# OpenDriveLab/ViDAR

Measured on AMD Instinct MI355X. Metric: train samples/sec (6-cam->BEV step), higher is better.
Workload: dtype f32

## Files before the change

### vidar_amd/csrc/gemm_mfma.hip

```cpp
#include <hip/hip_runtime.h>

#include <stdint.h>

#include "vidar_hip.h"
#include "vidar_common.h"

namespace {

typedef __bf16 bf16x8 __attribute__((ext_vector_type(8)));
typedef __bf16 bf16x2 __attribute__((ext_vector_type(2)));
typedef float f32x16 __attribute__((ext_vector_type(16)));
typedef float f32x2 __attribute__((ext_vector_type(2)));
typedef float f32x4 __attribute__((ext_vector_type(4)));
typedef float f32x4u __attribute__((ext_vector_type(4), aligned(4)));
typedef uint32_t u32x4 __attribute__((ext_vector_type(4)));
typedef uint32_t u32x2 __attribute__((ext_vector_type(2)));

constexpr int BM = 128, BN = 128, THREADS = 256;
constexpr int BK = 32;
constexpr int MN_STRIDE = 128 + 8;
template <int PREC>
struct Geo {
  static constexpr int UNITS = (PREC == 1) ? 16 : 32;
  static constexpr int KM_STRIDE = (PREC == 1) ? UNITS : UNITS + 4;
  static constexpr int IMG_DWORDS = (128 * KM_STRIDE > UNITS * MN_STRIDE) ? 128 * KM_STRIDE : UNITS * MN_STRIDE;
  static constexpr int NS = UNITS / 8;
};
constexpr int PREC_F32 = 0, PREC_BF16X3 = 1;
constexpr int LAY_K = 0, LAY_MN = 1;

struct GemmArgs {
  const float* A; const float* B; float* C;
  int64_t lda, ldb, ldc, sA, sB, sC;
  int M, N, K;
  int splits, k_chunk;
  int slabs;
  const float* scale; const float* shift; int vec_axis;
  const float* residual; int64_t ldr, sR;
  int relu;
  int tiles_m, tiles_n, m_fastest;
  int total;
  float* a_rowsum;
  float* rowsum_ws;
};

template <int PREC>
struct Staged {
  static constexpr int CH = 2;
  f32x4 v[CH][2];
};

template <int PREC>
struct KMap {
  static constexpr int LPR = 8;
  static constexpr int RPI = 64 / LPR;
  static constexpr int NI = 32 / RPI;
};

typedef uint32_t raw4 __attribute__((__vector_size__(4 * sizeof(uint32_t))));

__device__ __forceinline__ __amdgpu_buffer_rsrc_t make_rsrc(const float* p, int64_t bytes = 0x7fffffff) {
  const uint64_t a = (uint64_t)p;
  const uint32_t lo = __builtin_amdgcn_readfirstlane((uint32_t)a), hi = __builtin_amdgcn_readfirstlane((uint32_t)(a >> 32));
  const int32_t n = __builtin_amdgcn_readfirstlane((int32_t)(bytes > 0x7fffffff ? 0x7fffffff : bytes));
  return __builtin_amdgcn_make_buffer_rsrc((void*)(((uint64_t)hi << 32) | lo), 0, n, 0x00020000);
}
__device__ __forceinline__ f32x4 ld16(__amdgpu_buffer_rsrc_t r, uint32_t voff, uint32_t soff) {
  return __builtin_bit_cast(f32x4, __builtin_amdgcn_raw_buffer_load_b128(r, voff, soff, 0));
}
__device__ __forceinline__ float ld4(__amdgpu_buffer_rsrc_t r, uint32_t voff, uint32_t soff) {
  return __builtin_bit_cast(float, __builtin_amdgcn_raw_buffer_load_b32(r, voff, soff, 0));
}

template <int PREC>
__device__ __forceinline__ uint32_t voff_kmajor(int64_t ld, int tid) {
  using M = KMap<PREC>;
  const int lane = tid & 63, wave = tid >> 6;
  return (uint32_t)(((32 * wave + lane / M::LPR) * (uint32_t)ld + (lane % M::LPR) * 4) * 4);
}

template <int PREC>
__device__ __forceinline__ void load_kmajor(Staged<PREC>& s, __amdgpu_buffer_rsrc_t rs, int64_t ld, int krel, int k0, int kend,
                                            bool tail, int tid, uint32_t voff) {
  using M = KMap<PREC>;
#pragma unroll
  for (int i = 0; i < M::NI; ++i)
    s.v[i >> 1][i & 1] = ld16(rs, voff, (uint32_t)((i * M::RPI * (uint32_t)ld + krel) * 4));
  if (tail) {
    const int k = k0 + ((tid & 63) % M::LPR) * 4;
#pragma unroll
    for (int i = 0; i < M::NI; ++i)
#pragma unroll
      for (int j = 0; j < 4; ++j) s.v[i >> 1][i & 1][j] = (k + j < kend) ? s.v[i >> 1][i & 1][j] : 0.0f;
  }
}

template <int PREC>
__device__ __forceinline__ uint32_t voff_mnmajor(int64_t ld, int tid) {
  const int kr = (PREC == PREC_BF16X3) ? (tid >> 5) * 2 : (tid >> 5);
  return (uint32_t)((kr * (uint32_t)ld + (tid & 31) * 4) * 4);
}

template <int PREC>
__device__ __forceinline__ void load_mnmajor(Staged<PREC>& s, __amdgpu_buffer_rsrc_t rs, int64_t ld, int krel, uint32_t voff) {
#pragma unroll
  for (int i = 0; i < Staged<PREC>::CH * 2; ++i) {
    const int ku = (PREC == PREC_BF16X3) ? 16 * (i >> 1) + (i & 1) : 8 * i;
    s.v[i >> 1][i & 1] = ld16(rs, voff, (uint32_t)(krel + ku) * (uint32_t)ld * 4u);
  }
}

__device__ __forceinline__ void split2(float a, float b, uint32_t& hi, uint32_t& lo) {
  f32x2 x = {a, b};
  bf16x2 h = __builtin_convertvector(x, bf16x2);
  f32x2 r = x - __builtin_convertvector(h, f32x2);
  bf16x2 l = __builtin_convertvector(r, bf16x2);
  hi = __builtin_bit_cast(uint32_t, h);
  lo = __builtin_bit_cast(uint32_t, l);
}

template <int PREC>
__device__ __forceinline__ void store_kmajor(const Staged<PREC>& s, uint32_t* img, int tid) {
  using M = KMap<PREC>;
  const int lane = tid & 63, wave = tid >> 6;
  const int r0 = 32 * wave + lane / M::LPR, kq = lane % M::LPR;
#pragma unroll
  for (int i = 0; i < M::NI; ++i) {
    const int r = r0 + i * M::RPI;
    const f32x4 v = s.v[i >> 1][i & 1];
    if (PREC == PREC_BF16X3) {
      uint32_t h0, l0, h1, l1;
      split2(v[0], v[1], h0, l0);
      split2(v[2], v[3], h1, l1);
      const int pos = r * Geo<PREC>::KM_STRIDE + ((((kq >> 1) ^ ((r >> 2) & 3)) << 2) | ((kq & 1) << 1));
      *(u32x2*)(img + pos) = u32x2{h0, h1};
      *(u32x2*)(img + Geo<PREC>::IMG_DWORDS + pos) = u32x2{l0, l1};
    } else {
      *(u32x4*)(img + r * Geo<PREC>::KM_STRIDE + 4 * kq) = __builtin_bit_cast(u32x4, v);
    }
  }
}

template <int PREC>
__device__ __forceinline__ void store_mnmajor(const Staged<PREC>& s, uint32_t* img, int tid) {
  if (PREC == PREC_BF16X3) {
#pragma unroll
    for (int c = 0; c < 2; ++c) {
      const int item = tid + 256 * c;
      const int cq = (item & 31) * 4, u = item >> 5;
      u32x4 hi, lo;
#pragma unroll
      for (int j = 0; j < 4; ++j) {
        uint32_t h, l;
        split2(s.v[c][0][j], s.v[c][1][j], h, l);
        hi[j] = h; lo[j] = l;
      }
      *(u32x4*)(img + u * MN_STRIDE + cq) = hi;
      *(u32x4*)(img + Geo<PREC>::IMG_DWORDS + u * MN_STRIDE + cq) = lo;
    }
  } else {
#pragma unroll
    for (int i = 0; i < 4; ++i) {
      const int item = tid + 256 * i;
      *(u32x4*)(img + (item >> 5) * MN_STRIDE + (item & 31) * 4) = __builtin_bit_cast(u32x4, s.v[i >> 1][i & 1]);
    }
  }
}

template <int PREC, int LAY>
__device__ __forceinline__ u32x4 frag(const uint32_t* img, int row, int s, int h) {
  if (LAY == LAY_K) {
    if (PREC == PREC_BF16X3)
      return *(const u32x4*)(img + row * Geo<PREC>::KM_STRIDE + (((2 * s + h) ^ ((row >> 2) & 3)) << 2));
    return *(const u32x4*)(img + row * Geo<PREC>::KM_STRIDE + 8 * s + 4 * h);
  }
  u32x4 f;
  const uint32_t* p = img + (8 * s + 4 * h) * MN_STRIDE + row;
#pragma unroll
  for (int j = 0; j < 4; ++j) f[j] = p[j * MN_STRIDE];
  return f;
}

struct Tile {
  int z, batch, m0, n0, kbeg, kend;
  __amdgpu_buffer_rsrc_t rsA, rsB;
};

template <int PREC, int ALAY, int BLAY>
__device__ __forceinline__ Tile decode_tile(const GemmArgs& g, int t) {
  const int per_z = g.tiles_m * g.tiles_n;
  int id;
  {
    const int q = g.total >> 3, r = g.total & 7, x = t & 7;
    id = (x < r ? x * (q + 1) : r * (q + 1) + (x - r) * q) + (t >> 3);
  }
  Tile T;
  T.z = __builtin_amdgcn_readfirstlane(id / per_z);
  const int tt = id - T.z * per_z;
  const int tm = __builtin_amdgcn_readfirstlane(g.m_fastest ? tt % g.tiles_m : tt / g.tiles_n);
  const int tn = __builtin_amdgcn_readfirstlane(g.m_fastest ? tt / g.tiles_m : tt % g.tiles_n);
  T.batch = __builtin_amdgcn_readfirstlane(T.z / g.splits);
  const int split = T.z - T.batch * g.splits;
  T.m0 = tm * BM; T.n0 = tn * BN;
  T.kbeg = split * g.k_chunk;
  T.kend = min(g.K, T.kbeg + g.k_chunk);
  const float* A = g.A + (int64_t)T.batch * g.sA;
  const float* B = g.B + (int64_t)T.batch * g.sB;
  const int64_t kleft = g.K - T.kbeg;
  T.rsA = ALAY == LAY_K ? make_rsrc(A + (int64_t)T.m0 * g.lda + T.kbeg, ((int64_t)(g.M - 1 - T.m0) * g.lda + kleft) * 4)
                        : make_rsrc(A + (int64_t)T.kbeg * g.lda + T.m0, ((kleft - 1) * g.lda + (g.M - T.m0)) * 4);
  T.rsB = BLAY == LAY_K ? make_rsrc(B + (int64_t)T.n0 * g.ldb + T.kbeg, ((int64_t)(g.N - 1 - T.n0) * g.ldb + kleft) * 4)
                        : make_rsrc(B + (int64_t)T.kbeg * g.ldb + T.n0, ((kleft - 1) * g.ldb + (g.N - T.n0)) * 4);
  return T;
}

template <int PREC, int ALAY, int BLAY>
__device__ __forceinline__ void fetch(Staged<PREC>& sa, Staged<PREC>& sb, const GemmArgs& g, const Tile& T, int k0, int tid,
                                      uint32_t voa, uint32_t vob) {
  const int krel = k0 - T.kbeg;
  const bool tail = k0 + BK > T.kend;
  if (ALAY == LAY_K) load_kmajor<PREC>(sa, T.rsA, g.lda, krel, k0, T.kend, tail, tid, voa);
  else load_mnmajor<PREC>(sa, T.rsA, g.lda, krel, voa);
  if (BLAY == LAY_K) load_kmajor<PREC>(sb, T.rsB, g.ldb, krel, k0, T.kend, tail, tid, vob);
  else load_mnmajor<PREC>(sb, T.rsB, g.ldb, krel, vob);
}

template <int PREC>
__device__ __forceinline__ void add_rowsum(f32x4& rs, const Staged<PREC>& sa) {
#pragma unroll
  for (int i = 0; i < Staged<PREC>::CH * 2; ++i) rs += sa.v[i >> 1][i & 1];
}

template <int PREC, int ALAY, int BLAY>
__device__ __forceinline__ void mainloop(f32x16 (&acc)[2][2], Staged<PREC>& sa, Staged<PREC>& sb, const GemmArgs& g,
                                         const Tile& T, uint32_t* imgA, uint32_t* imgB, int tid, uint32_t voa, uint32_t vob,
                                         f32x4& rowsum, bool want_rowsum) {
  constexpr int IMGS = (PREC == PREC_BF16X3) ? 2 : 1;
  constexpr int IMG_DWORDS = Geo<PREC>::IMG_DWORDS;
  const int lane = tid & 63, wave = tid >> 6;
  const int wm = (wave >> 1) * 64, wn = (wave & 1) * 64;
  const int l31 = lane & 31, h = lane >> 5;
  for (int k0 = T.kbeg; k0 < T.kend; k0 += BK) {
    if (ALAY == LAY_MN && want_rowsum) add_rowsum<PREC>(rowsum, sa);
    if (ALAY == LAY_K) store_kmajor<PREC>(sa, imgA, tid); else store_mnmajor<PREC>(sa, imgA, tid);
    if (BLAY == LAY_K) store_kmajor<PREC>(sb, imgB, tid); else store_mnmajor<PREC>(sb, imgB, tid);
    __syncthreads();
    if (k0 + BK < T.kend) fetch<PREC, ALAY, BLAY>(sa, sb, g, T, k0 + BK, tid, voa, vob);
#pragma unroll
    for (int s = 0; s < Geo<PREC>::NS; ++s) {
      u32x4 fa[2][IMGS], fb[2][IMGS];
#pragma unroll
      for (int i = 0; i < 2; ++i)
#pragma unroll
        for (int p = 0; p < IMGS; ++p) {
          fa[i][p] = frag<PREC, ALAY>(imgA + p * IMG_DWORDS, wm + 32 * i + l31, s, h);
          fb[i][p] = frag<PREC, BLAY>(imgB + p * IMG_DWORDS, wn + 32 * i + l31, s, h);
        }
      if (PREC == PREC_BF16X3) {
#pragma unroll
        for (int term = 0; term < 3; ++term)
#pragma unroll
          for (int i = 0; i < 2; ++i)
#pragma unroll
            for (int j = 0; j < 2; ++j) {
              const bf16x8 a = __builtin_bit_cast(bf16x8, fa[i][term == 0 ? IMGS - 1 : 0]);
              const bf16x8 b = __builtin_bit_cast(bf16x8, fb[j][term == 1 ? IMGS - 1 : 0]);
              acc[i][j] = __builtin_amdgcn_mfma_f32_32x32x16_bf16(a, b, acc[i][j], 0, 0, 0);
            }
      } else {
#pragma unroll
        for (int u = 0; u < 4; ++u)
#pragma unroll
          for (int i = 0; i < 2; ++i)
#pragma unroll
            for (int j = 0; j < 2; ++j) {
              const f32x4 bf = __builtin_bit_cast(f32x4, fb[j][0]), af = __builtin_bit_cast(f32x4, fa[i][0]);
              acc[i][j] = __builtin_amdgcn_mfma_f32_32x32x2f32(af[u], bf[u], acc[i][j], 0, 0, 0);
            }
      }
    }
    __syncthreads();
  }
}

template <bool RAGGED_M>
__device__ __forceinline__ void epilogue_impl(const f32x16 (&acc)[2][2], const GemmArgs& g, const Tile& T, int tid) {
  const int lane = tid & 63, wave = tid >> 6;
  const int wm = (wave >> 1) * 64, wn = (wave & 1) * 64;
  const int l31 = lane & 31, h = lane >> 5;
  const int m0 = T.m0, n0 = T.n0;
  float* C; int64_t ldc;
  if (g.slabs) { C = g.C + (int64_t)T.z * g.M * g.N; ldc = g.N; }
  else { C = g.C + (int64_t)T.batch * g.sC; ldc = g.ldc; }
  const bool epi = !g.slabs;
  const bool by_n = epi && g.vec_axis == 0, by_m = epi && g.vec_axis == 1;
  const int rows_left = g.M - m0, cols_left = g.N - n0;
  const int mleft = rows_left - wm - 4 * h;
  const __amdgpu_buffer_rsrc_t rsC = make_rsrc(C + (int64_t)m0 * ldc + n0, ((int64_t)(rows_left - 1) * ldc + cols_left) * 4);
  const uint32_t voC = (uint32_t)(((wm + 4 * h) * (uint32_t)ldc + wn + l31) * 4);
  const bool has_res = epi && g.residual != nullptr;
  const float* Rp = has_res ? g.residual + (int64_t)T.batch * g.sR + (int64_t)m0 * g.ldr + n0 : C;
  const __amdgpu_buffer_rsrc_t rsR = make_rsrc(Rp, has_res ? ((int64_t)(rows_left - 1) * g.ldr + cols_left) * 4 : 0);
  const uint32_t voR = (uint32_t)(((wm + 4 * h) * (uint32_t)g.ldr + wn + l31) * 4);
  const bool m_scale = by_m && g.scale != nullptr, m_shift = by_m && g.shift != nullptr;
  const __amdgpu_buffer_rsrc_t rsS = make_rsrc(m_scale ? g.scale + m0 : C, m_scale ? (int64_t)rows_left * 4 : 0);
  const __amdgpu_buffer_rsrc_t rsH = make_rsrc(m_shift ? g.shift + m0 : C, m_shift ? (int64_t)rows_left * 4 : 0);
  const uint32_t voM = (uint32_t)((wm + 4 * h) * 4);
#pragma unroll
  for (int j = 0; j < 2; ++j) {
    const int n = n0 + wn + 32 * j + l31;
    if (n >= g.N) continue;
    float sn = 1.0f, bn = 0.0f;
    if (by_n && g.scale) sn = g.scale[n];
    if (by_n && g.shift) bn = g.shift[n];
#pragma unroll
    for (int i = 0; i < 2; ++i) {
#pragma unroll
      for (int r0 = 0; r0 < 16; r0 += 8) {
        float sc[8], sh[8], rs[8];
#pragma unroll
        for (int r = 0; r < 8; ++r) {
          const int row = 32 * i + (r & 3) + 8 * ((r0 + r) >> 2);
          sc[r] = m_scale ? ld4(rsS, voM, (uint32_t)(row * 4)) : sn;
          sh[r] = m_shift ? ld4(rsH, voM, (uint32_t)(row * 4)) : bn;
          rs[r] = has_res ? ld4(rsR, voR, (uint32_t)((row * (uint32_t)g.ldr + 32 * j) * 4)) : 0.0f;
        }
#pragma unroll
        for (int r = 0; r < 8; ++r) {
          const int row = 32 * i + (r & 3) + 8 * ((r0 + r) >> 2);
          float y = acc[i][j][r0 + r];
          if (epi) {
            y = y * sc[r] + sh[r] + rs[r];
            if (g.relu && !(y > 0.0f)) y = 0.0f;
          }
          if (!RAGGED_M || row < mleft)
            __builtin_amdgcn_raw_buffer_store_b32(__builtin_bit_cast(uint32_t, y), rsC, voC,
                                                    (uint32_t)((row * (uint32_t)ldc + 32 * j) * 4), 0);
        }
      }
    }
  }
}

__device__ __forceinline__ void epilogue(const f32x16 (&acc)[2][2], const GemmArgs& g, const Tile& T, int tid) {
  if (g.M - T.m0 >= BM) epilogue_impl<false>(acc, g, T, tid);
  else epilogue_impl<true>(acc, g, T, tid);
}

template <int PREC, int ALAY, int BLAY>
__global__ __launch_bounds__(THREADS, 3) void gemm_mfma_kernel(GemmArgs g) {
  constexpr int IMGS = (PREC == PREC_BF16X3) ? 2 : 1;
  __shared__ __attribute__((aligned(16))) uint32_t lds[2 * IMGS * Geo<PREC>::IMG_DWORDS];
  uint32_t* imgA = lds;
  uint32_t* imgB = lds + IMGS * Geo<PREC>::IMG_DWORDS;
  const int tid = threadIdx.x;
  const uint32_t voa = ALAY == LAY_K ? voff_kmajor<PREC>(g.lda, tid) : voff_mnmajor<PREC>(g.lda, tid);
  const uint32_t vob = BLAY == LAY_K ? voff_kmajor<PREC>(g.ldb, tid) : voff_mnmajor<PREC>(g.ldb, tid);
  Staged<PREC> sa, sb;
  int t = blockIdx.x;
  if (t >= g.total) return;
  Tile cur = decode_tile<PREC, ALAY, BLAY>(g, t);
  if (cur.kbeg < cur.kend) fetch<PREC, ALAY, BLAY>(sa, sb, g, cur, cur.kbeg, tid, voa, vob);
  for (;;) {
    f32x16 acc[2][2];
#pragma unroll
    for (int i = 0; i < 2; ++i)
#pragma unroll
      for (int j = 0; j < 2; ++j)
#pragma unroll
        for (int r = 0; r < 16; ++r) acc[i][j][r] = 0.0f;
    f32x4 rowsum = {0.f, 0.f, 0.f, 0.f};
    const bool want_rowsum = ALAY == LAY_MN && g.a_rowsum != nullptr && cur.n0 == 0;
    mainloop<PREC, ALAY, BLAY>(acc, sa, sb, g, cur, imgA, imgB, tid, voa, vob, rowsum, want_rowsum);
    if (want_rowsum) {
      float* red = reinterpret_cast<float*>(lds);
      const int quad = tid & 31, part = tid >> 5;
      *(f32x4*)(red + (part * 32 + quad) * 4) = rowsum;
      __syncthreads();
      if (tid < BM) {
        float sum = 0.f;
#pragma unroll
        for (int p8 = 0; p8 < 8; ++p8) sum += red[(p8 * 32 + (tid >> 2)) * 4 + (tid & 3)];
        if (cur.m0 + tid < g.M) g.rowsum_ws[(int64_t)cur.z * g.M + cur.m0 + tid] = sum;
      }
      __syncthreads();
    }
    const int tn = t + (int)gridDim.x;
    const bool more = tn < g.total;
    if (more) {
      const Tile nxt = decode_tile<PREC, ALAY, BLAY>(g, tn);
      if (nxt.kbeg < nxt.kend) fetch<PREC, ALAY, BLAY>(sa, sb, g, nxt, nxt.kbeg, tid, voa, vob);
    }
    epilogue(acc, g, cur, tid);
    if (!more) break;
    cur = decode_tile<PREC, ALAY, BLAY>(g, tn);
    t = tn;
  }
}

constexpr int WS_THREADS = 512;

__device__ __forceinline__ void lds_barrier() { asm volatile("s_waitcnt lgkmcnt(0)\n\ts_barrier" ::: "memory"); }

template <int PREC, int ALAY, int BLAY>
struct Cursor {
  int t;
  int k0;
  Tile T;
  __device__ __forceinline__ void start(const GemmArgs& g, int t0) {
    t = t0;
    while (t < g.total) {
      T = decode_tile<PREC, ALAY, BLAY>(g, t);
      if (T.kbeg < T.kend) break;
      t += (int)gridDim.x;
    }
    k0 = (t < g.total) ? T.kbeg : 0;
  }
  __device__ __forceinline__ bool valid(const GemmArgs& g) const { return t < g.total; }
  __device__ __forceinline__ void advance(const GemmArgs& g) {
    k0 += BK;
    if (k0 >= T.kend) start(g, t + (int)gridDim.x);
  }
};

template <int PREC, int ALAY, int BLAY>
__global__ __launch_bounds__(WS_THREADS, 2) void gemm_mfma_ws_kernel(GemmArgs g) {
  constexpr int IMGS = (PREC == PREC_BF16X3) ? 2 : 1;
  constexpr int IMG_DWORDS = Geo<PREC>::IMG_DWORDS;
  constexpr int STAGE_DWORDS = 2 * IMGS * IMG_DWORDS;
  __shared__ __attribute__((aligned(16))) uint32_t lds[2 * STAGE_DWORDS];
  const int tid = threadIdx.x;
  const int wave = __builtin_amdgcn_readfirstlane(tid >> 6);
  if ((int)blockIdx.x >= g.total) return;

  if (wave >= 4) {
    const int ptid = tid - 256;
    const uint32_t voa = ALAY == LAY_K ? voff_kmajor<PREC>(g.lda, ptid) : voff_mnmajor<PREC>(g.lda, ptid);
    const uint32_t vob = BLAY == LAY_K ? voff_kmajor<PREC>(g.ldb, ptid) : voff_mnmajor<PREC>(g.ldb, ptid);
    Staged<PREC> sa0, sb0, sa1, sb1;
    Cursor<PREC, ALAY, BLAY> rd;
    rd.start(g, (int)blockIdx.x);
    int steps = 0;
    for (int t = (int)blockIdx.x; t < g.total; t += (int)gridDim.x) {
      const Tile T = decode_tile<PREC, ALAY, BLAY>(g, t);
      steps += (T.kend > T.kbeg) ? (T.kend - T.kbeg + BK - 1) / BK : 0;
    }
    if (rd.valid(g)) { fetch<PREC, ALAY, BLAY>(sa0, sb0, g, rd.T, rd.k0, ptid, voa, vob); rd.advance(g); }
    if (rd.valid(g)) { fetch<PREC, ALAY, BLAY>(sa1, sb1, g, rd.T, rd.k0, ptid, voa, vob); rd.advance(g); }
    for (int gs = 0; gs < steps; gs += 2) {
      {
        uint32_t* imgA = lds;
        uint32_t* imgB = lds + IMGS * IMG_DWORDS;
        if (ALAY == LAY_K) store_kmajor<PREC>(sa0, imgA, ptid); else store_mnmajor<PREC>(sa0, imgA, ptid);
        if (BLAY == LAY_K) store_kmajor<PREC>(sb0, imgB, ptid); else store_mnmajor<PREC>(sb0, imgB, ptid);
        if (rd.valid(g)) { fetch<PREC, ALAY, BLAY>(sa0, sb0, g, rd.T, rd.k0, ptid, voa, vob); rd.advance(g); }
        lds_barrier();
      }
      if (gs + 1 < steps) {
        uint32_t* imgA = lds + STAGE_DWORDS;
        uint32_t* imgB = lds + STAGE_DWORDS + IMGS * IMG_DWORDS;
        if (ALAY == LAY_K) store_kmajor<PREC>(sa1, imgA, ptid); else store_mnmajor<PREC>(sa1, imgA, ptid);
        if (BLAY == LAY_K) store_kmajor<PREC>(sb1, imgB, ptid); else store_mnmajor<PREC>(sb1, imgB, ptid);
        if (rd.valid(g)) { fetch<PREC, ALAY, BLAY>(sa1, sb1, g, rd.T, rd.k0, ptid, voa, vob); rd.advance(g); }
        lds_barrier();
      }
    }
    return;
  }

  const int lane = tid & 63;
  const int wm = (wave >> 1) * 64, wn = (wave & 1) * 64;
  const int l31 = lane & 31, h = lane >> 5;
  int gs = 0;
  for (int t = (int)blockIdx.x; t < g.total; t += (int)gridDim.x) {
    const Tile T = decode_tile<PREC, ALAY, BLAY>(g, t);
    f32x16 acc[2][2];
#pragma unroll
    for (int i = 0; i < 2; ++i)
#pragma unroll
      for (int j = 0; j < 2; ++j)
#pragma unroll
        for (int r = 0; r < 16; ++r) acc[i][j][r] = 0.0f;
    for (int k0 = T.kbeg; k0 < T.kend; k0 += BK, ++gs) {
      lds_barrier();
      const uint32_t* imgA = lds + (gs & 1) * STAGE_DWORDS;
      const uint32_t* imgB = imgA + IMGS * IMG_DWORDS;
#pragma unroll
      for (int s = 0; s < Geo<PREC>::NS; ++s) {
        u32x4 fa[2][IMGS], fb[2][IMGS];
#pragma unroll
        for (int i = 0; i < 2; ++i)
#pragma unroll
          for (int p = 0; p < IMGS; ++p) {
            fa[i][p] = frag<PREC, ALAY>(imgA + p * IMG_DWORDS, wm + 32 * i + l31, s, h);
            fb[i][p] = frag<PREC, BLAY>(imgB + p * IMG_DWORDS, wn + 32 * i + l31, s, h);
          }
        if (PREC == PREC_BF16X3) {
#pragma unroll
          for (int term = 0; term < 3; ++term)
#pragma unroll
            for (int i = 0; i < 2; ++i)
#pragma unroll
              for (int j = 0; j < 2; ++j) {
                const bf16x8 a = __builtin_bit_cast(bf16x8, fa[i][term == 0 ? IMGS - 1 : 0]);
                const bf16x8 b = __builtin_bit_cast(bf16x8, fb[j][term == 1 ? IMGS - 1 : 0]);
                acc[i][j] = __builtin_amdgcn_mfma_f32_32x32x16_bf16(a, b, acc[i][j], 0, 0, 0);
              }
        } else {
#pragma unroll
          for (int u = 0; u < 4; ++u)
#pragma unroll
            for (int i = 0; i < 2; ++i)
#pragma unroll
              for (int j = 0; j < 2; ++j) {
                const f32x4 bf = __builtin_bit_cast(f32x4, fb[j][0]), af = __builtin_bit_cast(f32x4, fa[i][0]);
                acc[i][j] = __builtin_amdgcn_mfma_f32_32x32x2f32(af[u], bf[u], acc[i][j], 0, 0, 0);
              }
        }
      }
    }
    epilogue(acc, g, T, tid);
  }
}

__global__ __launch_bounds__(256) void gemm_slab_reduce_kernel(const float* __restrict__ ws, int Z, GemmArgs g) {
  __shared__ f32x4 part[4][64];
  if (g.a_rowsum != nullptr) {
    const int lane = threadIdx.x & 63;
    for (int m = (int)blockIdx.x * 4 + (threadIdx.x >> 6); m < g.M; m += (int)gridDim.x * 4) {
      float a = 0.f;
      for (int z = lane; z < Z; z += 64) a += g.rowsum_ws[(int64_t)z * g.M + m];
#pragma unroll
      for (int off = 32; off > 0; off >>= 1) a += __shfl_xor(a, off, 64);
      if (lane == 0) g.a_rowsum[m] = a;
    }
  }
  const int64_t total = (int64_t)g.M * g.N;
  const int64_t quads = total >> 2;
  const int col = threadIdx.x & 63, zg = threadIdx.x >> 6;
  for (int64_t q0 = (int64_t)blockIdx.x * 64; q0 < quads + 1; q0 += (int64_t)gridDim.x * 64) {
    const int64_t q = q0 + col;
    f32x4 a = {0.f, 0.f, 0.f, 0.f};
    if (q < quads) {
      for (int z = zg; z < Z; z += 4) a += *(const f32x4u*)(ws + (int64_t)z * total + 4 * q);
    } else if (q == quads) {
      for (int z = zg; z < Z; z += 4)
        for (int e = 0; e < (int)(total & 3); ++e) a[e] += ws[(int64_t)z * total + 4 * q + e];
    }
    part[zg][col] = a;
    __syncthreads();
    if (zg == 0 && q <= quads) {
      const f32x4 sum = ((part[0][col] + part[1][col]) + part[2][col]) + part[3][col];
      const int n_el = q < quads ? 4 : (int)(total & 3);
      for (int e = 0; e < n_el; ++e) {
        const int64_t idx = 4 * q + e;
        const int m = (int)(idx / g.N), n = (int)(idx - (int64_t)m * g.N);
        const int vi = g.vec_axis == 1 ? m : n;
        float y = sum[e] * (g.scale ? g.scale[vi] : 1.0f) + (g.shift ? g.shift[vi] : 0.0f);
        if (g.residual) y += g.residual[(int64_t)m * g.ldr + n];
        g.C[(int64_t)m * g.ldc + n] = (g.relu && !(y > 0.0f)) ? 0.0f : y;
      }
    }
    __syncthreads();
  }
}

template <int PREC>
void launch_ws(const GemmArgs& g, int a_layout, int b_layout, dim3 grid, hipStream_t st) {
  if (a_layout == LAY_K && b_layout == LAY_K) hipLaunchKernelGGL((gemm_mfma_ws_kernel<PREC, LAY_K, LAY_K>), grid, dim3(WS_THREADS), 0, st, g);
  else if (a_layout == LAY_K) hipLaunchKernelGGL((gemm_mfma_ws_kernel<PREC, LAY_K, LAY_MN>), grid, dim3(WS_THREADS), 0, st, g);
  else if (b_layout == LAY_K) hipLaunchKernelGGL((gemm_mfma_ws_kernel<PREC, LAY_MN, LAY_K>), grid, dim3(WS_THREADS), 0, st, g);
  else hipLaunchKernelGGL((gemm_mfma_ws_kernel<PREC, LAY_MN, LAY_MN>), grid, dim3(WS_THREADS), 0, st, g);
}

int g_gemm_variant = 0;

template <int PREC>
void launch(const GemmArgs& g, int a_layout, int b_layout, dim3 grid, hipStream_t st) {
  if (a_layout == LAY_K && b_layout == LAY_K) hipLaunchKernelGGL((gemm_mfma_kernel<PREC, LAY_K, LAY_K>), grid, dim3(THREADS), 0, st, g);
  else if (a_layout == LAY_K) hipLaunchKernelGGL((gemm_mfma_kernel<PREC, LAY_K, LAY_MN>), grid, dim3(THREADS), 0, st, g);
  else if (b_layout == LAY_K) hipLaunchKernelGGL((gemm_mfma_kernel<PREC, LAY_MN, LAY_K>), grid, dim3(THREADS), 0, st, g);
  else hipLaunchKernelGGL((gemm_mfma_kernel<PREC, LAY_MN, LAY_MN>), grid, dim3(THREADS), 0, st, g);
}

int num_cus() {
  static int cached[64] = {0};
  int dev = 0;
  if (hipGetDevice(&dev) != hipSuccess || dev < 0 || dev >= 64) return 256;
  if (cached[dev] == 0) {
    hipDeviceProp_t prop;
    cached[dev] = (hipGetDeviceProperties(&prop, dev) == hipSuccess && prop.multiProcessorCount > 0)
                      ? prop.multiProcessorCount : 256;
  }
  return cached[dev];
}

int pick_splits(int M, int N, int K, int batch, int bk) {
  const int tiles = ((M + BM - 1) / BM) * ((N + BN - 1) / BN) * batch;
  int s = (512 + tiles - 1) / tiles;
  const int max_s = (K + 4 * bk - 1) / (4 * bk);
  if (s > max_s) s = max_s;
  if (s < 1) s = 1;
  if (s > 256) s = 256;
  return s;
}

}

extern "C" {

int vidar_gemm_set_variant(int variant) {
  const int prev = g_gemm_variant;
  g_gemm_variant = (variant < 0 || variant > 2) ? 0 : variant;
  return prev;
}

int vidar_gemm_splits(int M, int N, int K, int batch, int precision, int reduce) {
  if (!reduce) return 1;
  return pick_splits(M, N, K, batch, BK);
}

size_t vidar_gemm_workspace_bytes(int M, int N, int K, int batch, int precision, int reduce) {
  if (!reduce) return 0;
  const int s = vidar_gemm_splits(M, N, K, batch, precision, reduce);
  const size_t Z = (size_t)batch * s;
  if (reduce == 1) return Z > 1 ? Z * (size_t)M * N * sizeof(float) : 0;
  return Z * ((size_t)M * N + M) * sizeof(float);
}

int vidar_gemm_f32(const float* A, int64_t lda, int a_layout, const float* B, int64_t ldb, int b_layout, float* C,
                   int64_t ldc, int M, int N, int K, int batch, int64_t strideA, int64_t strideB, int64_t strideC,
                   const float* scale, const float* shift, int vec_axis, const float* residual, int64_t ldr,
                   int64_t strideR, int relu, int precision, int reduce, float* a_rowsum, void* workspace,
                   size_t workspace_bytes, void* stream) {
  VIDAR_ENTER();
  if (a_rowsum != nullptr && !(reduce && a_layout == LAY_MN)) return VIDAR_ERR_BAD_ARG;
  if (A == nullptr || B == nullptr || C == nullptr || M <= 0 || N <= 0 || K <= 0 || batch <= 0) return VIDAR_ERR_BAD_ARG;
  if ((a_layout != LAY_K && a_layout != LAY_MN) || (b_layout != LAY_K && b_layout != LAY_MN)) return VIDAR_ERR_BAD_ARG;
  if (precision != PREC_F32 && precision != PREC_BF16X3) return VIDAR_ERR_BAD_ARG;
  if (vec_axis != 0 && vec_axis != 1) return VIDAR_ERR_BAD_ARG;
  if (lda < (a_layout == LAY_K ? K : M) || ldb < (b_layout == LAY_K ? K : N) || ldc < N) return VIDAR_ERR_BAD_ARG;
  if (residual != nullptr && (ldr < N || ldr >= (1 << 22))) return VIDAR_ERR_BAD_ARG;
  if (ldc >= (1 << 22)) return VIDAR_ERR_BAD_ARG;
  if (lda >= (1 << 22) || ldb >= (1 << 22)) return VIDAR_ERR_BAD_ARG;
  if ((a_layout == LAY_MN && (int64_t)K * lda >= (1LL << 29)) || (b_layout == LAY_MN && (int64_t)K * ldb >= (1LL << 29)))
    return VIDAR_ERR_BAD_ARG;
  hipStream_t st = (hipStream_t)stream;
  const int bk = BK;
  GemmArgs g;
  g.A = A; g.B = B; g.C = C;
  g.lda = lda; g.ldb = ldb; g.ldc = ldc; g.sA = strideA; g.sB = strideB; g.sC = strideC;
  g.M = M; g.N = N; g.K = K;
  g.scale = scale; g.shift = shift; g.vec_axis = vec_axis; g.residual = residual; g.ldr = ldr; g.sR = strideR;
  g.relu = relu;
  g.tiles_m = (M + BM - 1) / BM; g.tiles_n = (N + BN - 1) / BN;
  g.m_fastest = M < N;
  g.splits = reduce ? pick_splits(M, N, K, batch, bk) : 1;
  g.k_chunk = ((K + g.splits - 1) / g.splits + bk - 1) / bk * bk;
  const int Z = batch * g.splits;
  g.slabs = (reduce && (Z > 1 || a_rowsum != nullptr)) ? 1 : 0;
  g.a_rowsum = a_rowsum;
  g.rowsum_ws = nullptr;
  if ((int64_t)g.tiles_m * g.tiles_n * Z > 0x3fffffff) return VIDAR_ERR_BAD_ARG;
  g.total = g.tiles_m * g.tiles_n * Z;
  if (reduce && (strideC != 0 || strideR != 0) && batch > 1) return VIDAR_ERR_BAD_ARG;
  GemmArgs k = g;
  if (g.slabs) {
    const size_t need = (size_t)Z * ((size_t)M * N + (a_rowsum ? M : 0)) * sizeof(float);
    if (workspace == nullptr || workspace_bytes < need) return VIDAR_ERR_BAD_ARG;
    k.C = (float*)workspace;
    g.rowsum_ws = a_rowsum ? (float*)workspace + (size_t)Z * M * N : nullptr;
    k.rowsum_ws = g.rowsum_ws;
  }
  k.total = g.tiles_m * g.tiles_n * Z;
  if (g_gemm_variant >= 1 && a_rowsum == nullptr) {
    const int resident = num_cus() * g_gemm_variant / 8 * 8;
    dim3 grid(k.total > resident ? resident : k.total);
    if (precision == PREC_BF16X3) launch_ws<PREC_BF16X3>(k, a_layout, b_layout, grid, st);
    else launch_ws<PREC_F32>(k, a_layout, b_layout, grid, st);
  } else {
    const int resident = num_cus() * 3 / 8 * 8;
    dim3 grid(k.total > resident ? resident : k.total);
    if (precision == PREC_BF16X3) launch<PREC_BF16X3>(k, a_layout, b_layout, grid, st);
    else launch<PREC_F32>(k, a_layout, b_layout, grid, st);
  }
  if (g.slabs) {
    const int64_t total = (int64_t)M * N;
    int blocks = (int)((total / 4 + 1 + 63) / 64);
    if (blocks > 4096) blocks = 4096;
    hipLaunchKernelGGL(gemm_slab_reduce_kernel, dim3(blocks), dim3(256), 0, st, (const float*)workspace, Z, g);
  }
  return vidar_last_error();
}

}
```

Before: 2.925.

## Overlap last K-step MFMAs with epilogue stores in persistent f32 GEMM

```diff
diff --git a/vidar_amd/csrc/gemm_mfma.hip b/vidar_amd/csrc/gemm_mfma.hip
--- a/vidar_amd/csrc/gemm_mfma.hip
+++ b/vidar_amd/csrc/gemm_mfma.hip
@@ -233,14 +233,14 @@
 
 template <int PREC, int ALAY, int BLAY>
 __device__ __forceinline__ void mainloop(f32x16 (&acc)[2][2], Staged<PREC>& sa, Staged<PREC>& sb, const GemmArgs& g,
-                                         const Tile& T, uint32_t* imgA, uint32_t* imgB, int tid, uint32_t voa, uint32_t vob,
-                                         f32x4& rowsum, bool want_rowsum) {
+                                         const Tile& T, int kstop, uint32_t* imgA, uint32_t* imgB, int tid, uint32_t voa,
+                                         uint32_t vob, f32x4& rowsum, bool want_rowsum) {
   constexpr int IMGS = (PREC == PREC_BF16X3) ? 2 : 1;
   constexpr int IMG_DWORDS = Geo<PREC>::IMG_DWORDS;
   const int lane = tid & 63, wave = tid >> 6;
   const int wm = (wave >> 1) * 64, wn = (wave & 1) * 64;
   const int l31 = lane & 31, h = lane >> 5;
-  for (int k0 = T.kbeg; k0 < T.kend; k0 += BK) {
+  for (int k0 = T.kbeg; k0 < kstop; k0 += BK) {
     if (ALAY == LAY_MN && want_rowsum) add_rowsum<PREC>(rowsum, sa);
     if (ALAY == LAY_K) store_kmajor<PREC>(sa, imgA, tid); else store_mnmajor<PREC>(sa, imgA, tid);
     if (BLAY == LAY_K) store_kmajor<PREC>(sb, imgB, tid); else store_mnmajor<PREC>(sb, imgB, tid);
@@ -347,10 +347,92 @@
   else epilogue_impl<true>(acc, g, T, tid);
 }
 
+constexpr int TAB_DWORDS = 2 * (BM + BM);
+
+__device__ __forceinline__ void lds_barrier() { asm volatile("s_waitcnt lgkmcnt(0)\n\ts_barrier" ::: "memory"); }
+
+__device__ __forceinline__ bool piped_tile(const GemmArgs& g, const Tile& T) {
+  return !g.slabs && (g.vec_axis == 1 || (g.scale == nullptr && g.shift == nullptr)) && g.M - T.m0 >= BM &&
+         g.N - T.n0 >= BN && T.kbeg < T.kend;
+}
+
+__device__ __forceinline__ float table_value(const GemmArgs& g, const Tile& T, int tid) {
+  const float* v = tid < BM ? g.scale : g.shift;
+  float x = tid < BM ? 1.0f : 0.0f;
+  if (v != nullptr) x = v[T.m0 + (tid & (BM - 1))];
+  return x;
+}
+
+template <int ALAY, int BLAY>
+__device__ __forceinline__ void last_step_stage(const Staged<PREC_F32>& sa, const Staged<PREC_F32>& sb, uint32_t* imgA,
+                                                uint32_t* imgB, float* tab, float tabv, int tid) {
+  if (ALAY == LAY_K) store_kmajor<PREC_F32>(sa, imgA, tid); else store_mnmajor<PREC_F32>(sa, imgA, tid);
+  if (BLAY == LAY_K) store_kmajor<PREC_F32>(sb, imgB, tid); else store_mnmajor<PREC_F32>(sb, imgB, tid);
+  tab[tid] = tabv;
+  __syncthreads();
+}
+
+template <int ALAY, int BLAY>
+__device__ __forceinline__ void last_step_piped(f32x16 (&acc)[2][2], const GemmArgs& g, const Tile& T, const uint32_t* imgA,
+                                                const uint32_t* imgB, const float* tab, int tid0) {
+  constexpr int PREC = PREC_F32;
+  int tid = tid0;
+  asm volatile("" : "+v"(tid));
+  const int lane = tid & 63, wave = tid >> 6;
+  const int wm = (wave >> 1) * 64, wn = (wave & 1) * 64;
+  const int l31 = lane & 31, h = lane >> 5;
+  const __amdgpu_buffer_rsrc_t rsC = make_rsrc(g.C + (int64_t)T.batch * g.sC + (int64_t)T.m0 * g.ldc + T.n0,
+                                               ((int64_t)(BM - 1) * g.ldc + BN) * 4);
+  const uint32_t ldc = (uint32_t)g.ldc, ldr = (uint32_t)g.ldr;
+  const uint32_t voC = (uint32_t)(((wm + 4 * h) * ldc + wn + l31) * 4);
+  const bool has_res = g.residual != nullptr;
+  const __amdgpu_buffer_rsrc_t rsR =
+      make_rsrc(has_res ? g.residual + (int64_t)T.batch * g.sR + (int64_t)T.m0 * g.ldr + T.n0 : g.C,
+                has_res ? ((int64_t)(BM - 1) * g.ldr + BN) * 4 : 0);
+  const uint32_t voR = (uint32_t)(((wm + 4 * h) * ldr + wn + l31) * 4), voRz = has_res ? voR : 0u;
+  const uint32_t rb = has_res ? 4u : 0u;
+  const float* tsc = tab + wm + 4 * h;
+  const float* tsh = tsc + BM;
+  const bool relu = g.relu != 0;
+  float rs[16];
+#pragma unroll
+  for (int r = 0; r < 16; ++r) rs[r] = ld4(rsR, voRz, (uint32_t)((((r & 3) + 8 * (r >> 2)) * ldr) * rb));
+  __builtin_amdgcn_sched_barrier(0);
+#pragma unroll
+  for (int sub = 0; sub <= 4; ++sub) {
+    const int i = (sub >> 1) & 1, j = sub & 1;
+    const int pi = ((sub - 1) >> 1) & 1, pj = (sub - 1) & 1;
+    asm volatile("" ::: "memory");
+#pragma unroll
+    for (int s = 0; s < 4; ++s) {
+      f32x4 af = {0.f, 0.f, 0.f, 0.f}, bf = af;
+      if (sub < 4) {
+        af = __builtin_bit_cast(f32x4, frag<PREC, ALAY>(imgA, wm + 32 * i + l31, s, h));
+        bf = __builtin_bit_cast(f32x4, frag<PREC, BLAY>(imgB, wn + 32 * j + l31, s, h));
+      }
+#pragma unroll
+      for (int u = 0; u < 4; ++u) {
+        if (sub < 4) acc[i][j] = __builtin_amdgcn_mfma_f32_32x32x2f32(af[u], bf[u], acc[i][j], 0, 0, 0);
+        if (sub > 0) {
+          const int r = 4 * s + u;
+          const int prow = 32 * pi + 8 * s + u;
+          float y = acc[pi][pj][r] * tsc[prow] + tsh[prow] + rs[r];
+          if (relu && !(y > 0.0f)) y = 0.0f;
+          __builtin_amdgcn_raw_buffer_store_b32(__builtin_bit_cast(uint32_t, y), rsC, voC, (uint32_t)((prow * ldc + 32 * pj) * 4), 0);
+          if (sub < 4) rs[r] = ld4(rsR, voRz, (uint32_t)(((32 * i + 8 * s + u) * ldr + 32 * j) * rb));
+        }
+      }
+      __builtin_amdgcn_sched_barrier(0);
+    }
+    if (sub == 3) lds_barrier();
+  }
+}
+
 template <int PREC, int ALAY, int BLAY>
 __global__ __launch_bounds__(THREADS, 3) void gemm_mfma_kernel(GemmArgs g) {
   constexpr int IMGS = (PREC == PREC_BF16X3) ? 2 : 1;
-  __shared__ __attribute__((aligned(16))) uint32_t lds[2 * IMGS * Geo<PREC>::IMG_DWORDS];
+  constexpr int IMGS_DWORDS = 2 * IMGS * Geo<PREC>::IMG_DWORDS;
+  __shared__ __attribute__((aligned(16))) uint32_t lds[IMGS_DWORDS + (PREC == PREC_F32 && ALAY == LAY_K ? TAB_DWORDS : 0)];
   uint32_t* imgA = lds;
   uint32_t* imgB = lds + IMGS * Geo<PREC>::IMG_DWORDS;
   const int tid = threadIdx.x;
@@ -361,7 +443,7 @@
   if (t >= g.total) return;
   Tile cur = decode_tile<PREC, ALAY, BLAY>(g, t);
   if (cur.kbeg < cur.kend) fetch<PREC, ALAY, BLAY>(sa, sb, g, cur, cur.kbeg, tid, voa, vob);
-  for (;;) {
+  for (int parity = 0;; parity ^= 1) {
     f32x16 acc[2][2];
 #pragma unroll
     for (int i = 0; i < 2; ++i)
@@ -371,7 +453,18 @@
         for (int r = 0; r < 16; ++r) acc[i][j][r] = 0.0f;
     f32x4 rowsum = {0.f, 0.f, 0.f, 0.f};
     const bool want_rowsum = ALAY == LAY_MN && g.a_rowsum != nullptr && cur.n0 == 0;
-    mainloop<PREC, ALAY, BLAY>(acc, sa, sb, g, cur, imgA, imgB, tid, voa, vob, rowsum, want_rowsum);
+    const int tn = t + (int)gridDim.x;
+    const bool more = tn < g.total;
+    constexpr bool PIPED = PREC == PREC_F32 && ALAY == LAY_K;
+    const bool piped = PIPED && piped_tile(g, cur);
+    float tabv = 0.0f;
+    if (piped) tabv = table_value(g, cur, tid);
+    const int kstop = piped ? cur.kbeg + (cur.kend - cur.kbeg - 1) / BK * BK : cur.kend;
+    mainloop<PREC, ALAY, BLAY>(acc, sa, sb, g, cur, kstop, imgA, imgB, tid, voa, vob, rowsum, want_rowsum);
+    float* tab = reinterpret_cast<float*>(lds) + IMGS_DWORDS + parity * (TAB_DWORDS / 2);
+    if constexpr (PIPED) {
+      if (piped) last_step_stage<ALAY, BLAY>(sa, sb, imgA, imgB, tab, tabv, tid);
+    }
     if (want_rowsum) {
       float* red = reinterpret_cast<float*>(lds);
       const int quad = tid & 31, part = tid >> 5;
@@ -385,13 +478,16 @@
       }
       __syncthreads();
     }
-    const int tn = t + (int)gridDim.x;
-    const bool more = tn < g.total;
     if (more) {
       const Tile nxt = decode_tile<PREC, ALAY, BLAY>(g, tn);
       if (nxt.kbeg < nxt.kend) fetch<PREC, ALAY, BLAY>(sa, sb, g, nxt, nxt.kbeg, tid, voa, vob);
     }
-    epilogue(acc, g, cur, tid);
+    if constexpr (PIPED) {
+      if (piped) last_step_piped<ALAY, BLAY>(acc, g, cur, imgA, imgB, tab, tid);
+      else epilogue(acc, g, cur, tid);
+    } else {
+      epilogue(acc, g, cur, tid);
+    }
     if (!more) break;
     cur = decode_tile<PREC, ALAY, BLAY>(g, tn);
     t = tn;
@@ -399,8 +495,6 @@
 }
 
 constexpr int WS_THREADS = 512;
-
-__device__ __forceinline__ void lds_barrier() { asm volatile("s_waitcnt lgkmcnt(0)\n\ts_barrier" ::: "memory"); }
 
 template <int PREC, int ALAY, int BLAY>
 struct Cursor {
```

Result: faster. 2.959 (median of 6 runs) (+1.2%).
